# Chen-Suyi/PointRegGPT

Measured on AMD Instinct MI355X. Metric: generated point-cloud pairs/sec (node), 128x128 depth, 1000-step DDNM, higher is better.
Workload: dtype bf16; 1 GPU; configs[2]: full pipeline (SE(3) z-buffer reproject + MaskUnet + DDNM sampler + MaskUnet + f64 unproject); batch_per_gpu=64, image_size=128, transitions=1000, sampler=ancestral-ddnm, unet_dim=64, streams=2, parallelism=scene-sharded x1, no collectives, hipgraph=one captured transition (U-Net + update), replayed per step

## Files before the change

pointreggpt_amd/csrc/conv_c64.hip:

```cpp
#include <atomic>
#include <cstdlib>

#include "conv.h"

namespace prg {

typedef __attribute__((ext_vector_type(8))) __bf16 c64_bf16x8;
typedef __attribute__((ext_vector_type(16))) float c64_f32x16;
typedef __attribute__((ext_vector_type(4))) unsigned int c64_u32x4;
typedef __attribute__((ext_vector_type(8))) _Float16 c64_f16x8;

namespace {

constexpr int TH = 8, TW = 32, HP = TW + 2, HALO = (TH + 2) * HP;
constexpr int ROWB = 144;
constexpr int NPT = 256;
constexpr int RPP = NPT / 8;
constexpr int KU = (HALO + RPP - 1) / RPP;
constexpr size_t AH_BYTES = (size_t)KU * RPP * ROWB;
constexpr size_t C64_LDS = 2 * AH_BYTES + 64 * sizeof(float);

__device__ inline float c64_lo(uint32_t w) { return __uint_as_float(w << 16); }
__device__ inline float c64_hi(uint32_t w) { return __uint_as_float(w & 0xffff0000u); }
__device__ inline uint32_t c64_pack(float a, float b) {
// ... 110 lines not shown
      for (int c = 0; c < 4; ++c) {
        const bf16_t* const wsrc = PRO == 3 ? reinterpret_cast<const bf16_t*>(L.w_f16) : L.w;
        const bf16_t* p = wsrc + ((size_t)(tap * d.kchunks + (c >> 1)) * d.CoutPad + wn * 32 + l31) * 32 + (c & 1) * 16 + hi * 8;
        wf[tap][c] = *reinterpret_cast<const c64_bf16x8*>(p);
      }
    float* const bias_lds = reinterpret_cast<float*>(smem + 2 * AH_BYTES);
    if (tid < 64) bias_lds[tid] = L.bias[tid];
    const float* const biasp = bias_lds + wn * 32 + 4 * hi;
    const int gn_per = fuse_stats ? (64 / L.gn_groups) >> 3 : 1;
    const unsigned x0off = (unsigned)(((wm * 4) * HP + l31) * ROWB + hi * 16);
    auto mma = [](const c64_bf16x8& a, const c64_bf16x8& b, const c64_f32x16& c) -> c64_f32x16 {
      if constexpr (PRO == 3)
        return __builtin_amdgcn_mfma_f32_32x32x16_f16(__builtin_bit_cast(c64_f16x8, a), __builtin_bit_cast(c64_f16x8, b), c, 0, 0, 0);
      else
        return __builtin_amdgcn_mfma_f32_32x32x16_bf16(a, b, c, 0, 0, 0);
    };
    c64_barrier();
    for (int s = 0; s < nsteps; ++s) {
      const char* const xb = smem + (size_t)(s & 1) * AH_BYTES + x0off;
      c64_f32x16 acc[4];
#pragma unroll
      for (int q = 0; q < 4; ++q) {
        const float4 b4 = *reinterpret_cast<const float4*>(biasp + 8 * q);
#pragma unroll
        for (int pt = 0; pt < 4; ++pt) { acc[pt][4 * q] = b4.x; acc[pt][4 * q + 1] = b4.y; acc[pt][4 * q + 2] = b4.z; acc[pt][4 * q + 3] = b4.w; }
      }
      constexpr int FD = 3, FR = 4, NF = 72;
      c64_bf16x8 fr[FR];
      auto foff = [](int n) { return ((n / 12) * HP + (n / 4) % 3) * ROWB + (n & 3) * 32; };
#pragma unroll
      for (int j = 0; j < FD && j < NF; ++j) fr[j] = *reinterpret_cast<const c64_bf16x8*>(xb + foff(j));
#pragma unroll
      for (int n = 0; n < NF; ++n) {
        const int r = n / 12, dx = (n / 4) % 3, c = n & 3;
        if (n + FD < NF) fr[(n + FD) % FR] = *reinterpret_cast<const c64_bf16x8*>(xb + foff(n + FD));
#pragma unroll
        for (int dy = 0; dy < 3; ++dy) {
          const int pt = r - dy;
          if (pt >= 0 && pt < 4) acc[pt] = mma(wf[dy * 3 + dx][c], fr[n % FR], acc[pt]);
        }
        __builtin_amdgcn_sched_barrier(0);
      }
      int tb, ty0, tx0;
      c64_tile(first + s * stride, tiles_x, tiles_y, tb, ty0, tx0);
      if (fuse_stats && L.gn_tickets) asm volatile("s_waitcnt vmcnt(0)" ::: "memory");
      c64_barrier();
      float V[8];
#pragma unroll
      for (int q = 0; q < 4; ++q) {
        V[q] = 0.0f;
        V[4 + q] = 0.0f;
      }
      char* const obase = reinterpret_cast<char*>(L.out) +
                          ((((size_t)tb * d.Hout + ty0 + wm * 4) * d.Wout + tx0 + l31) * 64 + wn * 32 + 8 * hi) * 2;
      const size_t orow = (size_t)d.Wout * 128;
#pragma unroll
      for (int pt = 0; pt < 4; ++pt) {
        uint32_t pk[8];
#pragma unroll
        for (int q = 0; q < 4; ++q) {
          float v[4];
#pragma unroll
          for (int r = 0; r < 4; ++r) {
            v[r] = acc[pt][4 * q + r];
            V[q] += v[r];
            V[4 + q] = fmaf(v[r], v[r], V[4 + q]);
          }
          pk[2 * q] = O16 ? h16_pack(v[0], v[1]) : c64_pack(v[0], v[1]);
          pk[2 * q + 1] = O16 ? h16_pack(v[2], v[3]) : c64_pack(v[2], v[3]);
        }
#pragma unroll
        for (int m = 0; m < 2; ++m) {
          const auto s0 = __builtin_amdgcn_permlane32_swap(pk[4 * m], pk[4 * m + 2], false, false);
          const auto s1 = __builtin_amdgcn_permlane32_swap(pk[4 * m + 1], pk[4 * m + 3], false, false);
          const c64_u32x4 o = {(uint32_t)s0[0], (uint32_t)s1[0], (uint32_t)s0[1], (uint32_t)s1[1]};
          *reinterpret_cast<c64_u32x4*>(obase + pt * orow + m * 32) = o;
        }
      }
      if (fuse_stats) {
        const bool b0 = lane & 1, b1 = lane & 2, b2 = lane & 4;
        float A4[4], B2[2];
#pragma unroll
        for (int j = 0; j < 4; ++j) A4[j] = (b0 ? V[4 + j] : V[j]) + c64_dpp<0xB1>(b0 ? V[j] : V[4 + j]);
#pragma unroll
        for (int j = 0; j < 2; ++j) B2[j] = (b1 ? A4[2 + j] : A4[j]) + c64_dpp<0x4E>(b1 ? A4[j] : A4[2 + j]);
        float D = (b2 ? B2[1] : B2[0]) + c64_swz<4>(b2 ? B2[0] : B2[1]);
        D += c64_swz<8>(D);
        D += c64_swz<16>(D);
        D += __shfl_xor(D, 32, 64);
        const int per = gn_per > 4 ? 4 : gn_per;
        if (per >= 2) D += c64_swz<4>(D);
        if (per >= 4) D += c64_dpp<0x4E>(D);
        const int i = (lane & 1) * 4 + (lane & 2) + ((lane >> 2) & 1);
        const int q = i & 3;
        if (lane < 8 && (q & (per - 1)) == 0) {
          const int split_n = gn_per > 4 ? 2 : 1;
          const int nsplit = tiles_x * tiles_y * 2 * split_n;
          const int slab = (((ty0 / TH) * tiles_x + tx0 / TW) * 2 + wm) * split_n + (split_n == 2 ? wn : 0);
          const int grp = (wn * 4 + q) / gn_per;
          if (L.gn_acc) {
            int which = i >> 2;
            asm volatile("" : "+v"(which));
            gn_acc_add(L.gn_acc, L.gn_groups, tb, grp, which, D);
          } else {
            __hip_atomic_store(&L.gn_partials[(((size_t)tb * nsplit + slab) * L.gn_groups + grp) * 2 + (i >> 2)], D,
                               __ATOMIC_RELAXED, __HIP_MEMORY_SCOPE_AGENT);
          }
        }
      }
    }
    if (fuse_stats && L.gn_tickets) asm volatile("s_waitcnt vmcnt(0)" ::: "memory");
    if (nsteps & 1) c64_barrier();
    c64_barrier();
    return;
  }

  {
    const int ptid = tid - 256;
    const int slot = ptid & 7, row = ptid >> 3;
    char* const ah = smem + row * ROWB + slot * 16;
    const int Hl = d.Hout, Wl = d.Wout;
    int voffk[KU];
    unsigned m_valid = 0, m_top = 0, m_bot = 0, m_left = 0, m_right = 0;
#pragma unroll
    for (int k = 0; k < KU; ++k) {
      const int hp = k * RPP + row;
      const int hy = hp / HP, hx = hp - hy * HP;
      const bool valid = hp < HALO;
      const int dy = (hy - 1) >> d.ups, dx = (hx - 1) >> d.ups;
      voffk[k] = ((dy + 1) * d.Win + dx + 1) * 128 + slot * 16;
      m_valid |= (valid ? 1u : 0u) << k;
      m_top |= (valid && hy == 0 ? 1u : 0u) << k;
      m_bot |= (valid && hy == TH + 1 ? 1u : 0u) << k;
      m_left |= (valid && hx == 0 ? 1u : 0u) << k;
      m_right |= (valid && hx == HP - 1 ? 1u : 0u) << k;
    }
    const unsigned pad_bytes = (unsigned)(d.Win + 1) * 128u;
    const __amdgpu_buffer_rsrc_t rsrc = __builtin_amdgcn_make_buffer_rsrc(
        const_cast<char*>(reinterpret_cast<const char*>(L.src0)) - pad_bytes, 0,
        (int)((size_t)d.B * d.Hin * d.Win * 128 + pad_bytes), 0x00020000);
    c64_u32x4 hA[KU], hB[KU];
    const int tpi = tiles_x * tiles_y;
    int done_in_img = 0;
    unsigned okmask = 0, okmask_nxt = 0;
    float4 ca[2], cb[2], ca_n[2], cb_n[2];
    h16x2 ah2[4], bh2[4];
    longlong2 fs_n = make_longlong2(0, 0);
    auto issue = [&](int s, c64_u32x4(&h)[KU]) {
      int b, y0, x0;
      c64_tile(first + min(s, nsteps - 1) * stride, tiles_x, tiles_y, b, y0, x0);
      okmask_nxt = m_valid & ~((y0 == 0 ? m_top : 0u) | (y0 + TH == Hl ? m_bot : 0u) | (x0 == 0 ? m_left : 0u) |
                               (x0 + TW == Wl ? m_right : 0u));
      const int soff = __builtin_amdgcn_readfirstlane((((b * d.Hin + (y0 >> d.ups)) * d.Win) + (x0 >> d.ups)) * 128);
#pragma unroll
      for (int k = 0; k < KU; ++k)
        h[k] = __builtin_amdgcn_raw_buffer_load_b128(rsrc, ((okmask_nxt >> k) & 1u) ? voffk[k] : -1, soff, 0);
      if constexpr (PRO == 1) {
        const float* pa = L.pro_a + (size_t)b * 64 + slot * 8;
        const float* pb = L.pro_b + (size_t)b * 64 + slot * 8;
        ca_n[0] = *reinterpret_cast<const float4*>(pa);
        ca_n[1] = *reinterpret_cast<const float4*>(pa + 4);
        cb_n[0] = *reinterpret_cast<const float4*>(pb);
        cb_n[1] = *reinterpret_cast<const float4*>(pb + 4);
      }
      if constexpr (PRO >= 2) {
        const GnFold& f = L.pro_fold;
        fs_n = *reinterpret_cast<const longlong2*>(f.acc + ((size_t)b * f.G + (slot * 8) / f.cpg) * 2);
        const float* pp = f.P + (size_t)b * f.pq_stride + slot * 8;
        const float* pq = f.Q + (size_t)b * f.pq_stride + slot * 8;
        ca_n[0] = *reinterpret_cast<const float4*>(pp);
        ca_n[1] = *reinterpret_cast<const float4*>(pp + 4);
        cb_n[0] = *reinterpret_cast<const float4*>(pq);
        cb_n[1] = *reinterpret_cast<const float4*>(pq + 4);
      }
    };
    auto write = [&](int s, c64_u32x4(&h)[KU]) {
      char* dst = ah + (size_t)(s & 1) * AH_BYTES;
      const float a8[8] = {ca[0].x, ca[0].y, ca[0].z, ca[0].w, ca[1].x, ca[1].y, ca[1].z, ca[1].w};
      const float b8[8] = {cb[0].x, cb[0].y, cb[0].z, cb[0].w, cb[1].x, cb[1].y, cb[1].z, cb[1].w};
#pragma unroll
      for (int k = 0; k < KU; ++k) {
        c64_u32x4 v = h[k];
        if constexpr (PRO == 3) {
          v = h16_silu8(v, ah2, bh2);
        } else if constexpr (PRO) {
#pragma unroll
          for (int j = 0; j < 4; ++j) {
            const float lo = c64_silu(fmaf(c64_lo(v[j]), a8[2 * j], b8[2 * j]));
            const float hh = c64_silu(fmaf(c64_hi(v[j]), a8[2 * j + 1], b8[2 * j + 1]));
            v[j] = c64_pack(lo, hh);
          }
        }
        if constexpr (PRO != 0) {
          if (!((okmask >> k) & 1u)) v = c64_u32x4{0u, 0u, 0u, 0u};
        }
        *reinterpret_cast<c64_u32x4*>(dst + k * RPP * ROWB) = v;
      }
    };
    auto adopt = [&]() {
      okmask = okmask_nxt;
      if constexpr (PRO == 1) {
        ca[0] = ca_n[0]; ca[1] = ca_n[1]; cb[0] = cb_n[0]; cb[1] = cb_n[1];
      }
      if constexpr (PRO >= 2) {
        float mean, rstd;
        gn_fold_stats_raw(fs_n.x, fs_n.y, L.pro_fold.inv_n, mean, rstd);
#pragma unroll
        for (int h2 = 0; h2 < 2; ++h2) {
          ca[h2] = make_float4(rstd * ca_n[h2].x, rstd * ca_n[h2].y, rstd * ca_n[h2].z, rstd * ca_n[h2].w);
          cb[h2] = make_float4(fmaf(-mean, ca[h2].x, cb_n[h2].x), fmaf(-mean, ca[h2].y, cb_n[h2].y),
                               fmaf(-mean, ca[h2].z, cb_n[h2].z), fmaf(-mean, ca[h2].w, cb_n[h2].w));
        }
        if constexpr (PRO == 3) {
          typedef __attribute__((ext_vector_type(2))) float f32x2;
#pragma unroll
          for (int h2 = 0; h2 < 2; ++h2) {
            ah2[2 * h2] = __builtin_convertvector((f32x2){ca[h2].x, ca[h2].y}, h16x2);
            ah2[2 * h2 + 1] = __builtin_convertvector((f32x2){ca[h2].z, ca[h2].w}, h16x2);
            bh2[2 * h2] = __builtin_convertvector((f32x2){cb[h2].x, cb[h2].y}, h16x2);
            bh2[2 * h2 + 1] = __builtin_convertvector((f32x2){cb[h2].z, cb[h2].w}, h16x2);
          }
        }
      }
    };
    issue(0, hA);
    adopt();
    write(0, hA);
    issue(1, hB);
    c64_barrier();
    auto ticket = [&](int s) {
      if (fuse_stats && L.gn_tickets && ptid < 64) {
        const int t = first + s * stride;
        const int img = t / tpi;
        ++done_in_img;
        const bool leave = s + 1 == nsteps || (t + stride) / tpi != img;
        if (leave) {
          int old = 0;
          if (ptid == 0) old = __hip_atomic_fetch_add(L.gn_tickets + img, done_in_img, __ATOMIC_RELAXED, __HIP_MEMORY_SCOPE_AGENT);
          old = __builtin_amdgcn_readfirstlane(old);
          if (old + done_in_img == tpi) {
            if (ptid == 0) __hip_atomic_store(L.gn_tickets + img, 0, __ATOMIC_RELAXED, __HIP_MEMORY_SCOPE_AGENT);
            c64_fold_coefficients(L, img, tpi * 2 * (((64 / L.gn_groups) >> 3) > 4 ? 2 : 1), ptid);
          }
          done_in_img = 0;
        }
      }
    };
    const int n2 = (nsteps + 1) & ~1;
#pragma unroll 1
    for (int s = 0; s < n2; s += 2) {
      adopt();
      issue(s + 2, hA);
      write(s + 1, hB);
      c64_barrier();
      if (s > 0) ticket(s - 1);
      adopt();
      issue(s + 3, hB);
      write(s + 2, hA);
      c64_barrier();
      if (s < nsteps) ticket(s);
    }
    c64_barrier();
    if (n2 == nsteps) ticket(nsteps - 1);
  }
}

}

int try_launch_conv3x3_c64(const ConvLaunch<bf16_t>& L, hipStream_t s, int* gn_nsplit_out, int* acc_done) {
  static const int enabled = env_int("PRG_CONV_C64", 1);
  if (!enabled) return 0;
  const ConvDesc& d = L.d;
  if (!(d.KH == 3 && d.KW == 3 && d.stride == 1 && d.pad == 1)) return 0;
  if (d.C0 != 64 || d.C1 != 0 || d.Cout != 64 || d.CoutPad != 64 || d.kchunks != 2) return 0;
  if (L.residual || !L.bias) return 0;
  if (d.ups) return 0;
  if (d.Wout % TW || d.Hout % TH) return 0;
  if ((size_t)d.B * d.Hin * d.Win * 128 + 4096 >= ((size_t)1 << 31)) return 0;
  const int tiles_x = d.Wout / TW, tiles_y = d.Hout / TH;
  const int total = tiles_x * tiles_y * d.B;
  const int num_cus = device_cu_count();
  if (num_cus <= 0) return 0;
  int grid = (total < num_cus ? total : num_cus) & ~7;
  if (grid < 8) return 0;
  const int cpg = L.gn_groups > 0 ? 64 / L.gn_groups : 0;
  const int split_n = cpg > 32 ? 2 : 1;
  int fuse = L.gn_partials != nullptr && cpg % 8 == 0 && cpg <= 64 && (cpg & (cpg - 1)) == 0 &&
             tiles_x * tiles_y * 2 * split_n <= kGnMaxSplit;
  if (L.gn_partials && !fuse) return 0;
  static DeviceOnce attr_done[5];
  const GnFold& pf = L.pro_fold;
  const bool fold_ok = pf.acc && pf.P && pf.Q && pf.G * pf.cpg == 64 && pf.cpg % 8 == 0;
  if (pf.acc && !fold_ok) return 0;
  if (L.in_f16 && !(fold_ok && L.w_f16)) return 0;
  const int pro = L.in_f16 ? 3 : fold_ok ? 2 : (L.pro_a ? 1 : 0);
  if (L.out_f16 && pro != 0) return 0;
  const int variant = L.out_f16 ? 4 : pro;
  const void* const fns[5] = {reinterpret_cast<const void*>(&conv3x3_c64_kernel<0, false>), reinterpret_cast<const void*>(&conv3x3_c64_kernel<1, false>),
                              reinterpret_cast<const void*>(&conv3x3_c64_kernel<2, false>), reinterpret_cast<const void*>(&conv3x3_c64_kernel<3, false>),
                              reinterpret_cast<const void*>(&conv3x3_c64_kernel<0, true>)};
  if (!attr_done[variant].done()) {
    hipError_t e = hipFuncSetAttribute(fns[variant], hipFuncAttributeMaxDynamicSharedMemorySize, (int)C64_LDS);
    if (e != hipSuccess) return fail(PRG_E_HIP, std::string("hipFuncSetAttribute(c64 conv): ") + hipGetErrorString(e));
    attr_done[variant].mark();
  }
  if (gn_nsplit_out) *gn_nsplit_out = fuse ? tiles_x * tiles_y * 2 * split_n : 0;
  const bool use_acc = fuse && L.gn_acc != nullptr;
  ConvLaunch<bf16_t> Lk = L;
  Lk.gn_tickets = nullptr;
  if (!use_acc) Lk.gn_acc = nullptr;
  if (acc_done) *acc_done = use_acc ? 1 : 0;
  const int flags = (fuse ? 1 : 0) | 2;
  if (L.probe) return 1;
  if (variant == 4) conv3x3_c64_kernel<0, true><<<dim3(grid), 512, C64_LDS, s>>>(Lk, tiles_x, tiles_y, flags);
  else if (pro == 3) conv3x3_c64_kernel<3, false><<<dim3(grid), 512, C64_LDS, s>>>(Lk, tiles_x, tiles_y, flags);
  else if (pro == 2) conv3x3_c64_kernel<2, false><<<dim3(grid), 512, C64_LDS, s>>>(Lk, tiles_x, tiles_y, flags);
  else if (pro == 1) conv3x3_c64_kernel<1, false><<<dim3(grid), 512, C64_LDS, s>>>(Lk, tiles_x, tiles_y, flags);
  else conv3x3_c64_kernel<0, false><<<dim3(grid), 512, C64_LDS, s>>>(Lk, tiles_x, tiles_y, flags);
  PRG_LAUNCH_CHECK();
  return 1;
}

}
```

pointreggpt_amd/csrc/conv_ws.hip:

```cpp
#include <atomic>

#include "conv.h"

namespace prg {

typedef __attribute__((ext_vector_type(8))) __bf16 bf16x8;
typedef __attribute__((ext_vector_type(16))) float f32x16;
typedef __attribute__((ext_vector_type(4))) unsigned int u32x4;

namespace {

constexpr int kCH = 64;

__device__ inline float bf_lo(uint32_t w) { return __uint_as_float(w << 16); }
__device__ inline float bf_hi(uint32_t w) { return __uint_as_float(w & 0xffff0000u); }
__device__ inline uint32_t pack_bf16(float a, float b) {
  typedef __attribute__((ext_vector_type(2))) __bf16 bf16x2;
  bf16x2 v = {(__bf16)a, (__bf16)b};
  return __builtin_bit_cast(uint32_t, v);
}
template <int CTRL>
__device__ inline float dpp_f32(float v) {
  return __builtin_bit_cast(float, __builtin_amdgcn_update_dpp(0, __builtin_bit_cast(int, v), CTRL, 0xF, 0xF, false));
}
template <int XOR>
__device__ inline float swz_xor(float v) {
  return __builtin_bit_cast(float, __builtin_amdgcn_ds_swizzle(__builtin_bit_cast(int, v), (XOR << 10) | 0x1F));
}
__device__ inline float fast_silu(float x) {
  return x * __builtin_amdgcn_rcpf(1.0f + __builtin_amdgcn_exp2f(x * -1.4426950408889634f));
}

template <bool LDS_DONE = true>
__device__ __forceinline__ void phase_barrier() {
  if constexpr (LDS_DONE) asm volatile("s_waitcnt lgkmcnt(0)" ::: "memory");
  __builtin_amdgcn_s_barrier();
  asm volatile("" ::: "memory");
}

template <int TH, int TW, int BN>
struct WsGeom {
  static constexpr int BM = TH * TW;
  static constexpr int HP = TW + 2;
  static constexpr int HALO = (TH + 2) * HP;
  static constexpr int WAVES_N = BN / 64, WAVES_M = 4 / WAVES_N;
  static constexpr int ROWB = 144;
  static constexpr size_t AH_BYTES = (size_t)HALO * ROWB;
  static constexpr size_t BW_BYTES = (size_t)BN * ROWB;
  static constexpr size_t RED_BYTES = 0;
  static constexpr size_t STG_BYTES = 4 * 64 * 128;
  static constexpr size_t BIAS_BYTES = BN * sizeof(float);
  static constexpr size_t LDS = 2 * AH_BYTES + 3 * BW_BYTES + RED_BYTES + STG_BYTES + BIAS_BYTES;
  static_assert(LDS <= 160 * 1024, "LDS budget");
  static_assert(BM / WAVES_M == 64, "consumer wave tile is 64 pixels x 64 channels");
};

struct TileCur { int n, x, y, b; };

struct TileMap {
  int tiles_x, tiles_y, tiles_n, TH, TW;
  int pinned, tn_fixed;
  int first, stride, count;
  TileCur c0, dc;

  __device__ __forceinline__ void digits(int t, TileCur& c) const {
    if (pinned) {
      c.n = 0;
    } else {
      c.n = t % tiles_n;
      t /= tiles_n;
    }
    c.x = t % tiles_x; t /= tiles_x;
    c.y = t % tiles_y;
    c.b = t / tiles_y;
  }
  __device__ __forceinline__ void next(TileCur& c) const {
    int carry = 0;
    if (!pinned) {
      c.n += dc.n;
      if (c.n >= tiles_n) { c.n -= tiles_n; carry = 1; }
    }
    c.x += dc.x + carry; carry = 0;
    if (c.x >= tiles_x) { c.x -= tiles_x; carry = 1; }
    c.y += dc.y + carry; carry = 0;
    if (c.y >= tiles_y) { c.y -= tiles_y; carry = 1; }
    c.b += dc.b + carry;
  }
  __device__ __forceinline__ void fill(const TileCur& c, int& b, int& y0, int& x0, int& tn) const {
    b = c.b; y0 = c.y * TH; x0 = c.x * TW;
    tn = pinned ? tn_fixed : c.n;
  }

  __device__ __forceinline__ void init(int bid, int GR, int tx, int ty, int tn, int nb, int th, int tw) {
    tiles_x = tx; tiles_y = ty; tiles_n = tn; TH = th; TW = tw;
    const int npix = tx * ty * nb;
    const bool xcd_ok = (GR & 7) == 0;
    const int per_xcd = GR >> 3;
    const int xcd = bid & 7, idx = bid >> 3;
    if (xcd_ok && tn > 1 && (8 % tn) == 0) {
      pinned = 1;
      tn_fixed = xcd % tn;
      const int gx = 8 / tn, member = xcd / tn;
      first = member * per_xcd + idx;
      stride = gx * per_xcd;
      count = first < npix ? (npix - first + stride - 1) / stride : 0;
    } else {
      pinned = 0;
      tn_fixed = 0;
      first = xcd_ok ? xcd * per_xcd + idx : bid;
      stride = GR;
      const int total = npix * tn;
      count = first < total ? (total - first + stride - 1) / stride : 0;
    }
    digits(first, c0);
    digits(stride, dc);
  }
  __device__ __forceinline__ void decode(int it, int& b, int& y0, int& x0, int& tn) const {
    int t = first + it * stride;
    if (pinned) {
      tn = tn_fixed;
    } else {
      tn = t % tiles_n;
      t /= tiles_n;
    }
    const int tx = t % tiles_x; t /= tiles_x;
    const int ty = t % tiles_y;
    b = t / tiles_y;
    y0 = ty * TH; x0 = tx * TW;
  }
};

template <int TH, int TW, int BN, bool PRO>
struct Producer {
  using G = WsGeom<TH, TW, BN>;
  static constexpr int HP = G::HP, HALO = G::HALO;
  static constexpr int NPT = 512;
  static constexpr int NWL = BN * 8 / NPT;
  static constexpr int RPP = NPT / 8;
  static constexpr int DRAIN_PHASES = 2048 / NPT;
  static constexpr int KU = (HALO + RPP - 1) / RPP;
  static constexpr int UPH = (KU + 7) / 8 > 2 ? (KU + 7) / 8 : 2;
  static constexpr int NCO = PRO ? 4 : 0;
  static constexpr int PER_STEP = 9 * NWL + KU + NCO;
  static constexpr int U_YOUNGER = PER_STEP - 1;
  static_assert(U_YOUNGER <= 63, "vmcnt range");
  static constexpr int n_units(int p) {
    p = ((p % 9) + 9) % 9;
    if (p == 8) return 0;
    const int lo = p * UPH, hi = (p + 1) * UPH < KU ? (p + 1) * UPH : KU;
    return hi > lo ? hi - lo : 0;
  }
  static constexpr int n_coef(int p) { return ((p % 9) + 9) % 9 == 0 ? NCO : 0; }
  static constexpr int WD = 6;
  static constexpr int w_younger(int ph) {
    int n = n_units(ph - WD) + n_coef(ph);
    for (int j = 1; j < WD; ++j) n += n_coef(ph - j) + NWL + n_units(ph - j);
    return n;
  }
  static_assert(9 % 3 == 0 && 18 % WD == 0, "set index must be a compile-time function of (g & 1, phase)");

  const ConvLaunch<bf16_t>& L;
  const ConvDesc& d;
  const TileMap& tm;
  char* Ah0;
  char* Bw0;
  u32x4 wset[WD][NWL];
  u32x4 hreg[KU];
  u32x4 cf[2][4];
  unsigned hpix[KU];
  unsigned w_voff;
  unsigned cf_voff;
  unsigned dr_voff;
  unsigned hedge[KU];
  unsigned hvalid, hvalid_nxt;
  const char* ld_base;
  unsigned ld_cs2;
  unsigned ld_dummy;
  const char* ld_ca;
  const char* ld_cb;
  unsigned ld_tedge;
  int slot, row, nsteps, nchunks, Hl, Wl;
  struct StepInfo { int chunk, b, y0, x0, tn; TileCur cur; };
  StepInfo sA, sB, sC, dr;
  int gC;
  bool drain_on;
  const char* wptr;
  size_t w_tapb;
  char* dr_base;
  size_t dr_rowb;
  char* stage_rd;
  int dr_r0;

  __device__ __forceinline__ Producer(const ConvLaunch<bf16_t>& L_, char* smem, int ptid, const TileMap& tm_, int nsteps_,
                                      int nchunks_)
      : L(L_), d(L_.d), tm(tm_), nsteps(nsteps_), nchunks(nchunks_) {
    Ah0 = smem + (ptid >> 3) * G::ROWB + (ptid & 7) * 16;
    Bw0 = smem + 2 * G::AH_BYTES + (ptid >> 3) * G::ROWB + (ptid & 7) * 16;
    slot = ptid & 7;
    row = ptid >> 3;
    Hl = d.Hout;
    Wl = d.Wout;
    hvalid = hvalid_nxt = 0;
    ld_ca = ld_cb = nullptr;
    drain_on = false;
    w_tapb = (size_t)d.kchunks * d.CoutPad * 64;
    dr_rowb = (size_t)d.Wout * d.Cout * 2;
    dr_base = nullptr;
    wptr = nullptr;
    dr_r0 = ptid >> 3;
    stage_rd = smem + 2 * G::AH_BYTES + 3 * G::BW_BYTES + G::RED_BYTES + dr_r0 * 128 + (((ptid & 7) ^ ((dr_r0 >> 1) & 7)) << 4);
    sA.chunk = 0;
    sA.cur = tm.c0;
    tm.fill(sA.cur, sA.b, sA.y0, sA.x0, sA.tn);
    sB = sA; gC = 0;
    advance(sB);
    sC = sB;
    advance(sC);
    dr = sA;
    w_voff = (unsigned)((((slot >> 2) * d.CoutPad + row) * 32 + (slot & 3) * 8) * 2);
    cf_voff = (unsigned)(slot * 8 * 4);
    dr_voff = (unsigned)((((dr_r0 / TW) * d.Wout + dr_r0 % TW) * d.Cout + slot * 8) * 2);
    ld_dummy = (unsigned)((d.Win + 1));
#pragma unroll
    for (int k = 0; k < KU; ++k) {
      const int hp = k * RPP + row;
      const int hy = hp / HP, hx = hp - hy * HP;
      int ry = hy - 1, rx = hx - 1;
      if (d.ups) { ry >>= 1; rx >>= 1; }
      hpix[k] = (unsigned)((ry + 1) * d.Win + (rx + 1));
      hedge[k] = (hy == 0 ? 1u : 0u) | (hy == TH + 1 ? 2u : 0u) | (hx == 0 ? 4u : 0u) | (hx == TW + 1 ? 8u : 0u) |
                 (hp >= HALO ? 16u : 0u);
    }
  }

  __device__ __forceinline__ void advance(StepInfo& si) {
    if (gC + 1 < nsteps) {
      ++gC;
      if (++si.chunk == nchunks) {
        si.chunk = 0;
        tm.next(si.cur);
        tm.fill(si.cur, si.b, si.y0, si.x0, si.tn);
      }
    }
  }
  __device__ __forceinline__ const char* w_tile(int tap, int chunk, int tn) const {
    return reinterpret_cast<const char*>(L.w) + ((size_t)(tap * d.kchunks + 2 * chunk) * d.CoutPad + tn * BN) * 64;
  }
  template <int SET>
  __device__ __forceinline__ void w_issue(const char* base) {
    asm volatile("global_load_dwordx4 %0, %1, %2" : "=v"(wset[SET][0]) : "v"(w_voff), "s"(base) : "memory");
    if constexpr (NWL == 2) {
      const char* base2 = base + 4096;
      asm volatile("global_load_dwordx4 %0, %1, %2" : "=v"(wset[SET][NWL - 1]) : "v"(w_voff), "s"(base2) : "memory");
    }
  }
  template <int SET, int N>
  __device__ __forceinline__ void w_wait() {
    if constexpr (NWL == 2)
      asm volatile("s_waitcnt vmcnt(%[n])" : "+v"(wset[SET][0]), "+v"(wset[SET][1]) : [n] "i"(N) : "memory");
    else
      asm volatile("s_waitcnt vmcnt(%[n])" : "+v"(wset[SET][0]) : [n] "i"(N) : "memory");
    static_assert(NWL == 2 || NWL == 1, "weight units per thread");
  }
  template <int SET>
  __device__ __forceinline__ void w_write(int ring) {
#pragma unroll
    for (int j = 0; j < NWL; ++j)
      *reinterpret_cast<u32x4*>(Bw0 + ring * G::BW_BYTES + j * 64 * G::ROWB) = wset[SET][j];
  }

  __device__ __forceinline__ void issue_setup(const StepInfo& si) {
    const int b = si.b, y0 = si.y0, x0 = si.x0, chunk = si.chunk;
    const int c = chunk * kCH;
    const bool first = c < d.C0;
    const bf16_t* src = first ? L.src0 : L.src1;
    const int cs = first ? d.C0 : d.C1;
    const int cc = first ? c : c - d.C0;
    ld_cs2 = (unsigned)(cs * 2);
    ld_tedge = (y0 == 0 ? 1u : 0u) | (y0 + TH == Hl ? 2u : 0u) | (x0 == 0 ? 4u : 0u) | (x0 + TW == Wl ? 8u : 0u) | 16u;
    const int64_t horg = ((int64_t)b * d.Hin + (y0 >> d.ups)) * d.Win + (x0 >> d.ups) - (d.Win + 1);
    ld_base = reinterpret_cast<const char*>(src) + (horg * cs + cc) * 2;
    if constexpr (PRO) {
      const size_t o = ((size_t)b * d.C0 + chunk * kCH) * 4;
      ld_ca = reinterpret_cast<const char*>(L.pro_a) + o;
      ld_cb = reinterpret_cast<const char*>(L.pro_b) + o;
    }
    hvalid_nxt = 0;
  }
  template <int CS>
  __device__ __forceinline__ void issue_coeffs() {
    if constexpr (PRO) {
      asm volatile("global_load_dwordx4 %0, %1, %2" : "=v"(cf[CS][0]) : "v"(cf_voff), "s"(ld_ca) : "memory");
      asm volatile("global_load_dwordx4 %0, %1, %2 offset:16" : "=v"(cf[CS][1]) : "v"(cf_voff), "s"(ld_ca) : "memory");
      asm volatile("global_load_dwordx4 %0, %1, %2" : "=v"(cf[CS][2]) : "v"(cf_voff), "s"(ld_cb) : "memory");
      asm volatile("global_load_dwordx4 %0, %1, %2 offset:16" : "=v"(cf[CS][3]) : "v"(cf_voff), "s"(ld_cb) : "memory");
    }
  }
  template <int K>
  __device__ __forceinline__ void issue_unit() {
    const bool ok = (hedge[K] & ld_tedge) == 0;
    const unsigned pix = ok ? hpix[K] : ld_dummy;
    const unsigned voff = __umul24(pix, ld_cs2) + (unsigned)(slot * 16);
    asm volatile("global_load_dwordx4 %0, %1, %2" : "=v"(hreg[K]) : "v"(voff), "s"(ld_base) : "memory");
    hvalid_nxt |= (ok ? 1u : 0u) << K;
  }
  template <int K, int CS, int N>
  __device__ __forceinline__ void wait_unit() {
    if constexpr (PRO) {
      asm volatile("s_waitcnt vmcnt(%[n])"
                   : "+v"(hreg[K]), "+v"(cf[CS][0]), "+v"(cf[CS][1]), "+v"(cf[CS][2]), "+v"(cf[CS][3])
                   : [n] "i"(N)
                   : "memory");
    } else {
      asm volatile("s_waitcnt vmcnt(%[n])" : "+v"(hreg[K]) : [n] "i"(N) : "memory");
    }
  }
  template <int K, int CS>
  __device__ __forceinline__ void write_unit(int g_tgt, bool wr) {
    const int hp = K * RPP + row;
    if (hp < HALO && wr) {
      u32x4 v = hreg[K];
      if constexpr (PRO) {
#pragma unroll
        for (int j = 0; j < 4; ++j) {
          const float a_lo = __uint_as_float(cf[CS][j >> 1][(2 * j) & 3]);
          const float a_hi = __uint_as_float(cf[CS][j >> 1][((2 * j) & 3) + 1]);
          const float b_lo = __uint_as_float(cf[CS][2 + (j >> 1)][(2 * j) & 3]);
          const float b_hi = __uint_as_float(cf[CS][2 + (j >> 1)][((2 * j) & 3) + 1]);
          const float lo = fast_silu(fmaf(bf_lo(v[j]), a_lo, b_lo));
          const float hi2 = fast_silu(fmaf(bf_hi(v[j]), a_hi, b_hi));
          v[j] = pack_bf16(lo, hi2);
        }
      }
      if (!((hvalid >> K) & 1u)) v = u32x4{0u, 0u, 0u, 0u};
      *reinterpret_cast<u32x4*>(Ah0 + (g_tgt & 1) * G::AH_BYTES + K * RPP * G::ROWB) = v;
    }
  }
  template <int PH>
  __device__ __forceinline__ u32x4 drain_read() {
    return *reinterpret_cast<const u32x4*>(stage_rd + PH * 8192);
  }
  template <int PH>
  __device__ __forceinline__ void drain_store(const u32x4& v) {
    constexpr int wm = PH / G::WAVES_N, wn = PH % G::WAVES_N;
    constexpr int prow = (wm * 64) / TW;
    char* base = dr_base + prow * dr_rowb + wn * 128;
    asm volatile("global_store_dwordx4 %0, %1, %2" ::"v"(dr_voff), "v"(v), "s"(base) : "memory");
  }
  template <int PH>
  __device__ __forceinline__ void drain_unit() {
    drain_store<PH>(drain_read<PH>());
  }
  template <int PH, int J, int CSW>
  __device__ __forceinline__ void units_wait() {
    if constexpr (J < UPH && PH * UPH + J < KU) {
      wait_unit<PH * UPH + J, CSW, U_YOUNGER - NWL - J>();
      units_wait<PH, J + 1, CSW>();
    }
  }
  template <int PH, int J, int CSW>
  __device__ __forceinline__ void units_write(int g, bool wr) {
    if constexpr (J < UPH && PH * UPH + J < KU) {
      write_unit<PH * UPH + J, CSW>(g + 1, wr);
      units_write<PH, J + 1, CSW>(g, wr);
    }
  }
  template <int PH, int J>
  __device__ __forceinline__ void units_issue() {
    if constexpr (J < UPH && PH * UPH + J < KU) {
      issue_unit<PH * UPH + J>();
      units_issue<PH, J + 1>();
    }
  }
  template <int GP, int PH, bool LIVE>
  __device__ __forceinline__ void phase(int g, bool wr, int chunk0, int tn0, int chunk1, int tn1) {
    constexpr int SET = (3 * GP + PH + 2) % WD;
    constexpr int RING = (PH + 2) % 3;
    u32x4 dv;
    bool draining = false;
    if constexpr (LIVE && PH < DRAIN_PHASES) {
      draining = drain_on;
      if (draining) dv = drain_read<PH>();
    }
    if constexpr (LIVE || PH >= WD) {
      w_wait<SET, w_younger(PH)>();
      w_write<SET>(RING);
    }
    if constexpr (LIVE && PH < 8) {
      units_wait<PH, 0, (GP + 1) & 1>();
      units_write<PH, 0, (GP + 1) & 1>(g, wr);
    }
    constexpr int TAPN = PH + 2 + WD;
    static_assert(TAPN < 18, "weight prefetch reaches at most into the next step");
    if constexpr (!LIVE) wptr = TAPN < 9 ? w_tile(TAPN, chunk0, tn0) : w_tile(TAPN - 9, chunk1, tn1);
    else if constexpr (TAPN == 9) wptr = w_tile(0, chunk1, tn1);
    else wptr += w_tapb;
    w_issue<SET>(wptr);
    if constexpr (PH < 8) units_issue<PH, 0>();
    if constexpr (LIVE && PH < DRAIN_PHASES) {
      if (draining) drain_store<PH>(dv);
    }
    if constexpr (LIVE) phase_barrier();
  }
  template <int GP, bool LIVE>
  __device__ __forceinline__ void step(int g) {
    const bool wr = g + 1 < nsteps;
    if constexpr (LIVE) {
      const int c0 = sA.chunk, t0 = sA.tn, c1 = sB.chunk, t1 = sB.tn;
      drain_on = g > 0 && sA.chunk == 0;
      issue_coeffs<GP>();
      phase<GP, 0, LIVE>(g, wr, c0, t0, c1, t1); phase<GP, 1, LIVE>(g, wr, c0, t0, c1, t1);
      phase<GP, 2, LIVE>(g, wr, c0, t0, c1, t1); phase<GP, 3, LIVE>(g, wr, c0, t0, c1, t1);
      phase<GP, 4, LIVE>(g, wr, c0, t0, c1, t1); phase<GP, 5, LIVE>(g, wr, c0, t0, c1, t1);
      phase<GP, 6, LIVE>(g, wr, c0, t0, c1, t1); phase<GP, 7, LIVE>(g, wr, c0, t0, c1, t1);
      hvalid = hvalid_nxt;
      dr = sA;
      dr_base = reinterpret_cast<char*>(L.out) +
                ((((int64_t)dr.b * Hl + dr.y0) * Wl + dr.x0) * d.Cout + dr.tn * BN) * 2;
      sA = sB;
      sB = sC;
      advance(sC);
      issue_setup(sC);
      phase<GP, 8, LIVE>(g, wr, c0, t0, c1, t1);
    } else {
      const int c0 = sA.chunk, t0 = sA.tn;
      issue_setup(sB);
      issue_coeffs<GP>();
      phase<GP, 0, LIVE>(g, wr, c0, t0, c0, t0); phase<GP, 1, LIVE>(g, wr, c0, t0, c0, t0);
      phase<GP, 2, LIVE>(g, wr, c0, t0, c0, t0); phase<GP, 3, LIVE>(g, wr, c0, t0, c0, t0);
      phase<GP, 4, LIVE>(g, wr, c0, t0, c0, t0); phase<GP, 5, LIVE>(g, wr, c0, t0, c0, t0);
      phase<GP, 6, LIVE>(g, wr, c0, t0, c0, t0); phase<GP, 7, LIVE>(g, wr, c0, t0, c0, t0);
      phase<GP, 8, LIVE>(g, wr, c0, t0, c0, t0);
      hvalid = hvalid_nxt;
      issue_setup(sC);
    }
  }
  template <int K>
  __device__ __forceinline__ void prologue_issue() {
    if constexpr (K < KU) {
      issue_unit<K>();
      prologue_issue<K + 1>();
    }
  }
  template <int K>
  __device__ __forceinline__ void prologue_write() {
    if constexpr (K < KU) {
      wait_unit<K, 0, 0>();
      write_unit<K, 0>(0, true);
      prologue_write<K + 1>();
    }
  }
  __device__ __forceinline__ void prologue() {
    issue_setup(sA);
    issue_coeffs<0>();
    prologue_issue<0>();
    hvalid = hvalid_nxt;
    prologue_write<0>();
    step<1, false>(-1);
  }
  template <int K>
  __device__ __forceinline__ void keep_units() {
    if constexpr (K < KU) {
      asm volatile("" : "+v"(hreg[K])::"memory");
      keep_units<K + 1>();
    }
  }
  __device__ __forceinline__ void finish() {
    drain_unit<0>(); drain_unit<1>(); drain_unit<2>(); drain_unit<3>();
    static_assert(DRAIN_PHASES == 4, "one consumer wave's stage per drain phase");
    asm volatile("s_waitcnt vmcnt(0)" ::: "memory");
#pragma unroll
    for (int sidx = 0; sidx < WD; ++sidx)
#pragma unroll
      for (int j = 0; j < NWL; ++j) asm volatile("" : "+v"(wset[sidx][j])::"memory");
    keep_units<0>();
    if constexpr (PRO) {
#pragma unroll
      for (int c = 0; c < 2; ++c)
#pragma unroll
        for (int j = 0; j < 4; ++j) asm volatile("" : "+v"(cf[c][j])::"memory");
    }
    phase_barrier();
  }
};

template <int TH, int TW, int BN, bool PRO>
__global__ __launch_bounds__(768) void conv3x3_ws_kernel(const ConvLaunch<bf16_t> L, const int tiles_x,
                                                            const int tiles_y, const int tiles_n, const int fuse_stats) {
  using G = WsGeom<TH, TW, BN>;
  constexpr int HP = G::HP;
  extern __shared__ __attribute__((aligned(16))) char smem[];
  constexpr int ROWB = G::ROWB;
  char* const stage = smem + 2 * G::AH_BYTES + 3 * G::BW_BYTES + G::RED_BYTES;
  float* const bias_lds = reinterpret_cast<float*>(stage + G::STG_BYTES);

  const ConvDesc& d = L.d;
  const int tid = threadIdx.x, wave = tid >> 6, lane = tid & 63;
  const int nchunks = (d.C0 + d.C1) / kCH;
  TileMap tmap;
  tmap.init((int)blockIdx.x, (int)gridDim.x, tiles_x, tiles_y, tiles_n, d.B, TH, TW);
  const int my_tiles = tmap.count;
  const int nsteps = my_tiles * nchunks;
  if (nsteps == 0) return;

  if (wave < 4) {
    __builtin_amdgcn_s_setprio(3);
    const int gn_per = fuse_stats ? (d.Cout / L.gn_groups) >> 3 : 1;
    const int gn_per_sh = 31 - __builtin_clz(gn_per);
    const int wm = wave / G::WAVES_N, wn = wave % G::WAVES_N;
    const int l31 = lane & 31, hi = lane >> 5;
    const int lpx = (TW == 16 && l31 >= 16) ? 16 + ((l31 - 2) & 15) : l31;
    const char* xrow[2];
    const char* wrowp[2];
#pragma unroll
    for (int pt = 0; pt < 2; ++pt) {
      const int p = wm * 64 + pt * 32 + lpx;
      xrow[pt] = smem + ((p / TW) * HP + (p % TW)) * ROWB + hi * 16;
    }
#pragma unroll
    for (int ct = 0; ct < 2; ++ct) wrowp[ct] = smem + 2 * G::AH_BYTES + (wn * 64 + ct * 32 + l31) * ROWB + hi * 16;
    f32x16 acc[2][2];
#pragma unroll
    for (int ct = 0; ct < 2; ++ct)
#pragma unroll
      for (int pt = 0; pt < 2; ++pt)
#pragma unroll
        for (int e = 0; e < 16; ++e) acc[ct][pt][e] = 0.0f;

    if (tid < BN) bias_lds[tid] = L.bias[(tmap.pinned ? tmap.tn_fixed : 0) * BN + tid];
    phase_barrier<true>();
    bf16x8 fw[3][2], fx[3][2];
    const char* xa[2] = {xrow[0], xrow[1]};
    const char* xn[2] = {xrow[0] + G::AH_BYTES, xrow[1] + G::AH_BYTES};
#define PRG_LW(SET, CT, RING, CALL) fw[SET][CT] = *reinterpret_cast<const bf16x8*>(wrowp[CT] + (RING) * (int)G::BW_BYTES + (CALL) * 32)
#define PRG_LX(SET, PT, BASE, TOFF, CALL) fx[SET][PT] = *reinterpret_cast<const bf16x8*>(BASE[PT] + (TOFF) * ROWB + (CALL) * 32)
#define PRG_MM(SET, CT, PT) acc[CT][PT] = __builtin_amdgcn_mfma_f32_32x32x16_bf16(fw[SET][CT], fx[SET][PT], acc[CT][PT], 0, 0, 0)
#define PRG_SB() __builtin_amdgcn_sched_barrier(0)
    PRG_LW(0, 0, 0, 0); PRG_LX(0, 0, xa, 0, 0); PRG_LX(0, 1, xa, 0, 0); PRG_LW(0, 1, 0, 0);
    PRG_LW(1, 0, 0, 1); PRG_LX(1, 0, xa, 0, 1); PRG_LX(1, 1, xa, 0, 1); PRG_LW(1, 1, 0, 1);
    int chunk = 0, it = 0;
    int tb = 0, ty0 = 0, tx0 = 0, ttn = 0;
    TileCur tcur = tmap.c0;
    tmap.fill(tcur, tb, ty0, tx0, ttn);
    for (int g = 0; g < nsteps; ++g) {
      const bool tile_end = chunk == nchunks - 1;
#pragma unroll
      for (int p = 0; p < 9; ++p) {
        const int toff = (p / 3) * HP + (p % 3);
        const int pn = p == 8 ? 0 : p + 1;
        const int toffN = (pn / 3) * HP + (pn % 3);
#pragma unroll
        for (int call = 0; call < 4; ++call) {
          const int sl = (4 * p + call + 2) % 3, sm = (4 * p + call) % 3;
          if (call < 2) {
            PRG_LW(sl, 0, p % 3, call + 2); PRG_MM(sm, 0, 0); PRG_SB();
            PRG_LX(sl, 0, xa, toff, call + 2); PRG_MM(sm, 0, 1); PRG_SB();
            PRG_LX(sl, 1, xa, toff, call + 2); PRG_MM(sm, 1, 0); PRG_SB();
            PRG_LW(sl, 1, p % 3, call + 2); PRG_MM(sm, 1, 1); PRG_SB();
          } else if (p == 8) {
            PRG_LW(sl, 0, (p + 1) % 3, call - 2); PRG_MM(sm, 0, 0); PRG_SB();
            PRG_LX(sl, 0, xn, toffN, call - 2); PRG_MM(sm, 0, 1); PRG_SB();
            PRG_LX(sl, 1, xn, toffN, call - 2); PRG_MM(sm, 1, 0); PRG_SB();
            PRG_LW(sl, 1, (p + 1) % 3, call - 2); PRG_MM(sm, 1, 1); PRG_SB();
          } else {
            PRG_LW(sl, 0, (p + 1) % 3, call - 2); PRG_MM(sm, 0, 0); PRG_SB();
            PRG_LX(sl, 0, xa, toffN, call - 2); PRG_MM(sm, 0, 1); PRG_SB();
            PRG_LX(sl, 1, xa, toffN, call - 2); PRG_MM(sm, 1, 0); PRG_SB();
            PRG_LW(sl, 1, (p + 1) % 3, call - 2); PRG_MM(sm, 1, 1); PRG_SB();
          }
        }
        if (p == 8 && tile_end) {
          char* const stg = stage + wave * (64 * 128);
          float V[16];
          const bool o16 = L.out_f16 != 0;
#pragma unroll
          for (int ct = 0; ct < 2; ++ct)
#pragma unroll
            for (int q = 0; q < 4; ++q) {
              const float4 b4 = *reinterpret_cast<const float4*>(bias_lds + wn * 64 + ct * 32 + 8 * q + 4 * hi);
              const float bv[4] = {b4.x, b4.y, b4.z, b4.w};
              float s = 0.0f, sq = 0.0f;
#pragma unroll
              for (int pt = 0; pt < 2; ++pt) {
                float v[4];
#pragma unroll
                for (int r = 0; r < 4; ++r) {
                  v[r] = acc[ct][pt][4 * q + r] + bv[r];
                  s += v[r];
                  sq = fmaf(v[r], v[r], sq);
                }
                uint2 w;
                w.x = o16 ? h16_pack(v[0], v[1]) : pack_bf16(v[0], v[1]);
                w.y = o16 ? h16_pack(v[2], v[3]) : pack_bf16(v[2], v[3]);
                const int px = pt * 32 + lpx;
                *reinterpret_cast<uint2*>(stg + px * 128 + (((ct * 4 + q) ^ ((px >> 1) & 7)) << 4) + hi * 8) = w;
              }
              V[ct * 4 + q] = s;
              V[8 + ct * 4 + q] = sq;
            }
          if (fuse_stats) {
            const bool b0 = lane & 1, b1 = lane & 2, b2 = lane & 4, b3 = lane & 8;
            float A8[8], B4[4], C2[2];
#pragma unroll
            for (int j = 0; j < 8; ++j) A8[j] = (b0 ? V[8 + j] : V[j]) + dpp_f32<0xB1>(b0 ? V[j] : V[8 + j]);
#pragma unroll
            for (int j = 0; j < 4; ++j) B4[j] = (b1 ? A8[4 + j] : A8[j]) + dpp_f32<0x4E>(b1 ? A8[j] : A8[4 + j]);
#pragma unroll
            for (int j = 0; j < 2; ++j) C2[j] = (b2 ? B4[2 + j] : B4[j]) + swz_xor<4>(b2 ? B4[j] : B4[2 + j]);
            float D = (b3 ? C2[1] : C2[0]) + swz_xor<8>(b3 ? C2[0] : C2[1]);
            D += swz_xor<16>(D);
            D += __shfl_xor(D, 32, 64);
            const int per = gn_per;
            if (per >= 2) D += swz_xor<8>(D);
            if (per >= 4) D += swz_xor<4>(D);
            if (per >= 8) D += dpp_f32<0x4E>(D);
            const int i = (lane & 1) * 8 + (lane & 2) * 2 + ((lane >> 2) & 1) * 2 + ((lane >> 3) & 1);
            const int cc = i & 7;
            if (lane < 16 && (cc & (per - 1)) == 0) {
              const int nsplit = tiles_x * tiles_y * G::WAVES_M;
              const int slab = ((ty0 / TH) * tiles_x + tx0 / TW) * G::WAVES_M + wm;
              const int grp = (((ttn * BN + wn * 64) >> 3) + cc) >> gn_per_sh;
              if (L.gn_acc) gn_acc_add(L.gn_acc, L.gn_groups, tb, grp, i >> 3, D);
              else L.gn_partials[(((size_t)tb * nsplit + slab) * L.gn_groups + grp) * 2 + (i >> 3)] = D;
            }
          }
#pragma unroll
          for (int ct = 0; ct < 2; ++ct)
#pragma unroll
            for (int pt = 0; pt < 2; ++pt)
#pragma unroll
              for (int e = 0; e < 16; ++e) acc[ct][pt][e] = 0.0f;
        }
        if (p == 8 && tile_end) phase_barrier<true>();
        else phase_barrier<false>();
      }
      { const char* t0 = xa[0]; xa[0] = xn[0]; xn[0] = t0; const char* t1 = xa[1]; xa[1] = xn[1]; xn[1] = t1; }
      if (++chunk == nchunks) {
        chunk = 0;
        if (++it < my_tiles) {
          tmap.next(tcur);
          tmap.fill(tcur, tb, ty0, tx0, ttn);
        }
      }
    }
#undef PRG_LW
#undef PRG_LX
#undef PRG_MM
#undef PRG_SB
    phase_barrier<false>();
    return;
  }

  {
    Producer<TH, TW, BN, PRO> Pv(L, smem, tid - 256, tmap, nsteps, nchunks);
    Pv.prologue();
    phase_barrier();
#pragma unroll 1
    for (int g = 0; g < nsteps; g += 2) {
      Pv.template step<0, true>(g);
      if (g + 1 < nsteps) Pv.template step<1, true>(g + 1);
    }
    Pv.finish();
  }
}

constexpr int kWsUnsupported = 100;

template <int TH, int TW, int BN, bool PRO>
int launch_ws_cfg2(const ConvLaunch<bf16_t>& L, hipStream_t s, int fuse_stats, int* nsplit, int num_cus) {
  using G = WsGeom<TH, TW, BN>;
  const ConvDesc& d = L.d;
  const int tiles_x = d.Wout / TW, tiles_y = d.Hout / TH, tiles_n = d.Cout / BN;
  const int total = tiles_x * tiles_y * tiles_n * d.B;
  int grid = num_cus;
  if (grid > total) grid = total;
  if (grid >= 8) grid &= ~7;
  if (tiles_n > 1 && (grid & 7) != 0) return kWsUnsupported;
  static DeviceOnce attr_done;
  if (!attr_done.done()) {
    hipError_t e = hipFuncSetAttribute(reinterpret_cast<const void*>(&conv3x3_ws_kernel<TH, TW, BN, PRO>),
                                       hipFuncAttributeMaxDynamicSharedMemorySize, (int)G::LDS);
    if (e != hipSuccess) return fail(PRG_E_HIP, std::string("hipFuncSetAttribute(ws conv): ") + hipGetErrorString(e));
    attr_done.mark();
  }
  if (nsplit) *nsplit = fuse_stats ? tiles_x * tiles_y * G::WAVES_M : 0;
  if (L.probe) return PRG_OK;
  conv3x3_ws_kernel<TH, TW, BN, PRO><<<dim3(grid), 768, G::LDS, s>>>(L, tiles_x, tiles_y, tiles_n, fuse_stats);
  PRG_LAUNCH_CHECK();
  return PRG_OK;
}

template <int TH, int TW, int BN>
int launch_ws_cfg(const ConvLaunch<bf16_t>& L, hipStream_t s, int fuse_stats, int* nsplit, int num_cus) {
  return L.pro_a ? launch_ws_cfg2<TH, TW, BN, true>(L, s, fuse_stats, nsplit, num_cus)
                 : launch_ws_cfg2<TH, TW, BN, false>(L, s, fuse_stats, nsplit, num_cus);
}

}

int try_launch_conv3x3_ws(const ConvLaunch<bf16_t>& L, hipStream_t s, int* gn_nsplit_out, int* acc_done) {
  static const int enabled = env_int("PRG_CONV_WS", 1);
  if (!enabled) return 0;
  const ConvDesc& d = L.d;
  if (!(d.KH == 3 && d.KW == 3 && d.stride == 1 && d.pad == 1)) return 0;
  if (d.C0 % kCH || d.C1 % kCH || d.Cout % 64) return 0;
  if (L.residual || !L.bias) return 0;
  if (L.in_f16 || (L.out_f16 && L.pro_a)) return 0;
  {
    const int tn128 = d.Cout % 128 == 0 ? d.Cout / 128 : d.Cout / 64;
    if (tn128 != 1 && tn128 != 2 && tn128 != 4 && tn128 != 8) return 0;
  }
  const int num_cus = device_cu_count();
  if (num_cus <= 0) return 0;
  const int H = d.Hout, W = d.Wout;
  const int cpg = L.gn_groups > 0 ? d.Cout / L.gn_groups : 0;
  const bool want = L.gn_partials != nullptr;
  auto fuse_for = [&](int TH, int TW, int BN) {
    return want && cpg % 8 == 0 && cpg <= 64 && (cpg & (cpg - 1)) == 0 && (W / TW) * (H / TH) * (4 / (BN / 64)) <= kGnMaxSplit ? 1 : 0;
  };
  int rc = 0;
  if (d.Cout % 128 == 0) {
    if (W % 32 == 0 && H % 4 == 0) rc = launch_ws_cfg<4, 32, 128>(L, s, fuse_for(4, 32, 128), gn_nsplit_out, num_cus);
    else if (W % 16 == 0 && H % 8 == 0) rc = launch_ws_cfg<8, 16, 128>(L, s, fuse_for(8, 16, 128), gn_nsplit_out, num_cus);
    else return 0;
  } else {
    if (W % 32 == 0 && H % 8 == 0) rc = launch_ws_cfg<8, 32, 64>(L, s, fuse_for(8, 32, 64), gn_nsplit_out, num_cus);
    else return 0;
  }
  if (rc == kWsUnsupported) return 0;
  if (rc == PRG_OK && acc_done) *acc_done = (L.gn_acc && gn_nsplit_out && *gn_nsplit_out > 0) ? 1 : 0;
  return rc == PRG_OK ? 1 : rc;
}

}
```

Measured before the change: 14.55 pairs/s.

## Store conv epilogue directly from consumer waves via permlane32 swap, drop producer LDS drain

The warp-specialized conv epilogue used to stage bf16 outputs in an LDS buffer, which producer threads then drained to global memory over later phases. Consumer waves now pack their outputs, exchange halves across the wave with permlane32_swap, and write 16-byte chunks straight to global memory. This frees the staging LDS and removes the drain logic and the extra LDS wait at tile end. The trade is that consumers now spend time on global stores. Separately, the c64 kernel issues its halo buffer loads after the coefficient loads instead of before.

```diff
diff --git a/pointreggpt_amd/csrc/conv_c64.hip b/pointreggpt_amd/csrc/conv_c64.hip
--- a/pointreggpt_amd/csrc/conv_c64.hip
+++ b/pointreggpt_amd/csrc/conv_c64.hip
@@ -286,9 +286,6 @@
       okmask_nxt = m_valid & ~((y0 == 0 ? m_top : 0u) | (y0 + TH == Hl ? m_bot : 0u) | (x0 == 0 ? m_left : 0u) |
                                (x0 + TW == Wl ? m_right : 0u));
       const int soff = __builtin_amdgcn_readfirstlane((((b * d.Hin + (y0 >> d.ups)) * d.Win) + (x0 >> d.ups)) * 128);
-#pragma unroll
-      for (int k = 0; k < KU; ++k)
-        h[k] = __builtin_amdgcn_raw_buffer_load_b128(rsrc, ((okmask_nxt >> k) & 1u) ? voffk[k] : -1, soff, 0);
       if constexpr (PRO == 1) {
         const float* pa = L.pro_a + (size_t)b * 64 + slot * 8;
         const float* pb = L.pro_b + (size_t)b * 64 + slot * 8;
@@ -307,6 +304,9 @@
         cb_n[0] = *reinterpret_cast<const float4*>(pq);
         cb_n[1] = *reinterpret_cast<const float4*>(pq + 4);
       }
+#pragma unroll
+      for (int k = 0; k < KU; ++k)
+        h[k] = __builtin_amdgcn_raw_buffer_load_b128(rsrc, ((okmask_nxt >> k) & 1u) ? voffk[k] : -1, soff, 0);
     };
     auto write = [&](int s, c64_u32x4(&h)[KU]) {
       char* dst = ah + (size_t)(s & 1) * AH_BYTES;
diff --git a/pointreggpt_amd/csrc/conv_ws.hip b/pointreggpt_amd/csrc/conv_ws.hip
--- a/pointreggpt_amd/csrc/conv_ws.hip
+++ b/pointreggpt_amd/csrc/conv_ws.hip
@@ -47,10 +47,8 @@
   static constexpr int ROWB = 144;
   static constexpr size_t AH_BYTES = (size_t)HALO * ROWB;
   static constexpr size_t BW_BYTES = (size_t)BN * ROWB;
-  static constexpr size_t RED_BYTES = 0;
-  static constexpr size_t STG_BYTES = 4 * 64 * 128;
   static constexpr size_t BIAS_BYTES = BN * sizeof(float);
-  static constexpr size_t LDS = 2 * AH_BYTES + 3 * BW_BYTES + RED_BYTES + STG_BYTES + BIAS_BYTES;
+  static constexpr size_t LDS = 2 * AH_BYTES + 3 * BW_BYTES + BIAS_BYTES;
   static_assert(LDS <= 160 * 1024, "LDS budget");
   static_assert(BM / WAVES_M == 64, "consumer wave tile is 64 pixels x 64 channels");
 };
@@ -137,7 +135,6 @@
   static constexpr int NPT = 512;
   static constexpr int NWL = BN * 8 / NPT;
   static constexpr int RPP = NPT / 8;
-  static constexpr int DRAIN_PHASES = 2048 / NPT;
   static constexpr int KU = (HALO + RPP - 1) / RPP;
   static constexpr int UPH = (KU + 7) / 8 > 2 ? (KU + 7) / 8 : 2;
   static constexpr int NCO = PRO ? 4 : 0;
@@ -170,7 +167,6 @@
   unsigned hpix[KU];
   unsigned w_voff;
   unsigned cf_voff;
-  unsigned dr_voff;
   unsigned hedge[KU];
   unsigned hvalid, hvalid_nxt;
   const char* ld_base;
@@ -181,15 +177,10 @@
   unsigned ld_tedge;
   int slot, row, nsteps, nchunks, Hl, Wl;
   struct StepInfo { int chunk, b, y0, x0, tn; TileCur cur; };
-  StepInfo sA, sB, sC, dr;
+  StepInfo sA, sB, sC;
   int gC;
-  bool drain_on;
   const char* wptr;
   size_t w_tapb;
-  char* dr_base;
-  size_t dr_rowb;
-  char* stage_rd;
-  int dr_r0;
 
   __device__ __forceinline__ Producer(const ConvLaunch<bf16_t>& L_, char* smem, int ptid, const TileMap& tm_, int nsteps_,
                                       int nchunks_)
@@ -202,13 +193,8 @@
     Wl = d.Wout;
     hvalid = hvalid_nxt = 0;
     ld_ca = ld_cb = nullptr;
-    drain_on = false;
     w_tapb = (size_t)d.kchunks * d.CoutPad * 64;
-    dr_rowb = (size_t)d.Wout * d.Cout * 2;
-    dr_base = nullptr;
     wptr = nullptr;
-    dr_r0 = ptid >> 3;
-    stage_rd = smem + 2 * G::AH_BYTES + 3 * G::BW_BYTES + G::RED_BYTES + dr_r0 * 128 + (((ptid & 7) ^ ((dr_r0 >> 1) & 7)) << 4);
     sA.chunk = 0;
     sA.cur = tm.c0;
     tm.fill(sA.cur, sA.b, sA.y0, sA.x0, sA.tn);
@@ -216,10 +202,8 @@
     advance(sB);
     sC = sB;
     advance(sC);
-    dr = sA;
     w_voff = (unsigned)((((slot >> 2) * d.CoutPad + row) * 32 + (slot & 3) * 8) * 2);
     cf_voff = (unsigned)(slot * 8 * 4);
-    dr_voff = (unsigned)((((dr_r0 / TW) * d.Wout + dr_r0 % TW) * d.Cout + slot * 8) * 2);
     ld_dummy = (unsigned)((d.Win + 1));
 #pragma unroll
     for (int k = 0; k < KU; ++k) {
@@ -336,21 +320,6 @@
       *reinterpret_cast<u32x4*>(Ah0 + (g_tgt & 1) * G::AH_BYTES + K * RPP * G::ROWB) = v;
     }
   }
-  template <int PH>
-  __device__ __forceinline__ u32x4 drain_read() {
-    return *reinterpret_cast<const u32x4*>(stage_rd + PH * 8192);
-  }
-  template <int PH>
-  __device__ __forceinline__ void drain_store(const u32x4& v) {
-    constexpr int wm = PH / G::WAVES_N, wn = PH % G::WAVES_N;
-    constexpr int prow = (wm * 64) / TW;
-    char* base = dr_base + prow * dr_rowb + wn * 128;
-    asm volatile("global_store_dwordx4 %0, %1, %2" ::"v"(dr_voff), "v"(v), "s"(base) : "memory");
-  }
-  template <int PH>
-  __device__ __forceinline__ void drain_unit() {
-    drain_store<PH>(drain_read<PH>());
-  }
   template <int PH, int J, int CSW>
   __device__ __forceinline__ void units_wait() {
     if constexpr (J < UPH && PH * UPH + J < KU) {
@@ -376,12 +345,6 @@
   __device__ __forceinline__ void phase(int g, bool wr, int chunk0, int tn0, int chunk1, int tn1) {
     constexpr int SET = (3 * GP + PH + 2) % WD;
     constexpr int RING = (PH + 2) % 3;
-    u32x4 dv;
-    bool draining = false;
-    if constexpr (LIVE && PH < DRAIN_PHASES) {
-      draining = drain_on;
-      if (draining) dv = drain_read<PH>();
-    }
     if constexpr (LIVE || PH >= WD) {
       w_wait<SET, w_younger(PH)>();
       w_write<SET>(RING);
@@ -397,9 +360,6 @@
     else wptr += w_tapb;
     w_issue<SET>(wptr);
     if constexpr (PH < 8) units_issue<PH, 0>();
-    if constexpr (LIVE && PH < DRAIN_PHASES) {
-      if (draining) drain_store<PH>(dv);
-    }
     if constexpr (LIVE) phase_barrier();
   }
   template <int GP, bool LIVE>
@@ -407,16 +367,12 @@
     const bool wr = g + 1 < nsteps;
     if constexpr (LIVE) {
       const int c0 = sA.chunk, t0 = sA.tn, c1 = sB.chunk, t1 = sB.tn;
-      drain_on = g > 0 && sA.chunk == 0;
       issue_coeffs<GP>();
       phase<GP, 0, LIVE>(g, wr, c0, t0, c1, t1); phase<GP, 1, LIVE>(g, wr, c0, t0, c1, t1);
       phase<GP, 2, LIVE>(g, wr, c0, t0, c1, t1); phase<GP, 3, LIVE>(g, wr, c0, t0, c1, t1);
       phase<GP, 4, LIVE>(g, wr, c0, t0, c1, t1); phase<GP, 5, LIVE>(g, wr, c0, t0, c1, t1);
       phase<GP, 6, LIVE>(g, wr, c0, t0, c1, t1); phase<GP, 7, LIVE>(g, wr, c0, t0, c1, t1);
       hvalid = hvalid_nxt;
-      dr = sA;
-      dr_base = reinterpret_cast<char*>(L.out) +
-                ((((int64_t)dr.b * Hl + dr.y0) * Wl + dr.x0) * d.Cout + dr.tn * BN) * 2;
       sA = sB;
       sB = sC;
       advance(sC);
@@ -466,8 +422,6 @@
     }
   }
   __device__ __forceinline__ void finish() {
-    drain_unit<0>(); drain_unit<1>(); drain_unit<2>(); drain_unit<3>();
-    static_assert(DRAIN_PHASES == 4, "one consumer wave's stage per drain phase");
     asm volatile("s_waitcnt vmcnt(0)" ::: "memory");
 #pragma unroll
     for (int sidx = 0; sidx < WD; ++sidx)
@@ -491,8 +445,7 @@
   constexpr int HP = G::HP;
   extern __shared__ __attribute__((aligned(16))) char smem[];
   constexpr int ROWB = G::ROWB;
-  char* const stage = smem + 2 * G::AH_BYTES + 3 * G::BW_BYTES + G::RED_BYTES;
-  float* const bias_lds = reinterpret_cast<float*>(stage + G::STG_BYTES);
+  float* const bias_lds = reinterpret_cast<float*>(smem + 2 * G::AH_BYTES + 3 * G::BW_BYTES);
 
   const ConvDesc& d = L.d;
   const int tid = threadIdx.x, wave = tid >> 6, lane = tid & 63;
@@ -512,10 +465,12 @@
     const int lpx = (TW == 16 && l31 >= 16) ? 16 + ((l31 - 2) & 15) : l31;
     const char* xrow[2];
     const char* wrowp[2];
+    unsigned opix[2];
 #pragma unroll
     for (int pt = 0; pt < 2; ++pt) {
       const int p = wm * 64 + pt * 32 + lpx;
       xrow[pt] = smem + ((p / TW) * HP + (p % TW)) * ROWB + hi * 16;
+      opix[pt] = (unsigned)(((p / TW) * d.Wout + (p % TW)) * d.Cout * 2 + hi * 16);
     }
 #pragma unroll
     for (int ct = 0; ct < 2; ++ct) wrowp[ct] = smem + 2 * G::AH_BYTES + (wn * 64 + ct * 32 + l31) * ROWB + hi * 16;
@@ -570,33 +525,38 @@
           }
         }
         if (p == 8 && tile_end) {
-          char* const stg = stage + wave * (64 * 128);
           float V[16];
+#pragma unroll
+          for (int i = 0; i < 16; ++i) V[i] = 0.0f;
           const bool o16 = L.out_f16 != 0;
+          char* const obase = reinterpret_cast<char*>(L.out) +
+                              ((((size_t)tb * d.Hout + ty0) * d.Wout + tx0) * d.Cout + ttn * BN + wn * 64) * 2;
 #pragma unroll
           for (int ct = 0; ct < 2; ++ct)
 #pragma unroll
-            for (int q = 0; q < 4; ++q) {
-              const float4 b4 = *reinterpret_cast<const float4*>(bias_lds + wn * 64 + ct * 32 + 8 * q + 4 * hi);
-              const float bv[4] = {b4.x, b4.y, b4.z, b4.w};
-              float s = 0.0f, sq = 0.0f;
-#pragma unroll
-              for (int pt = 0; pt < 2; ++pt) {
+            for (int pt = 0; pt < 2; ++pt) {
+              uint32_t pk[8];
+#pragma unroll
+              for (int q = 0; q < 4; ++q) {
+                const float4 b4 = *reinterpret_cast<const float4*>(bias_lds + wn * 64 + ct * 32 + 8 * q + 4 * hi);
+                const float bv[4] = {b4.x, b4.y, b4.z, b4.w};
                 float v[4];
 #pragma unroll
                 for (int r = 0; r < 4; ++r) {
                   v[r] = acc[ct][pt][4 * q + r] + bv[r];
-                  s += v[r];
-                  sq = fmaf(v[r], v[r], sq);
+                  V[ct * 4 + q] += v[r];
+                  V[8 + ct * 4 + q] = fmaf(v[r], v[r], V[8 + ct * 4 + q]);
                 }
-                uint2 w;
-                w.x = o16 ? h16_pack(v[0], v[1]) : pack_bf16(v[0], v[1]);
-                w.y = o16 ? h16_pack(v[2], v[3]) : pack_bf16(v[2], v[3]);
-                const int px = pt * 32 + lpx;
-                *reinterpret_cast<uint2*>(stg + px * 128 + (((ct * 4 + q) ^ ((px >> 1) & 7)) << 4) + hi * 8) = w;
+                pk[2 * q] = o16 ? h16_pack(v[0], v[1]) : pack_bf16(v[0], v[1]);
+                pk[2 * q + 1] = o16 ? h16_pack(v[2], v[3]) : pack_bf16(v[2], v[3]);
               }
-              V[ct * 4 + q] = s;
-              V[8 + ct * 4 + q] = sq;
+#pragma unroll
+              for (int m = 0; m < 2; ++m) {
+                const auto s0 = __builtin_amdgcn_permlane32_swap(pk[4 * m], pk[4 * m + 2], false, false);
+                const auto s1 = __builtin_amdgcn_permlane32_swap(pk[4 * m + 1], pk[4 * m + 3], false, false);
+                const u32x4 o = {(uint32_t)s0[0], (uint32_t)s1[0], (uint32_t)s0[1], (uint32_t)s1[1]};
+                *reinterpret_cast<u32x4*>(obase + opix[pt] + ct * 64 + m * 32) = o;
+              }
             }
           if (fuse_stats) {
             const bool b0 = lane & 1, b1 = lane & 2, b2 = lane & 4, b3 = lane & 8;
@@ -631,8 +591,7 @@
 #pragma unroll
               for (int e = 0; e < 16; ++e) acc[ct][pt][e] = 0.0f;
         }
-        if (p == 8 && tile_end) phase_barrier<true>();
-        else phase_barrier<false>();
+        phase_barrier<false>();
       }
       { const char* t0 = xa[0]; xa[0] = xn[0]; xn[0] = t0; const char* t1 = xa[1]; xa[1] = xn[1]; xn[1] = t1; }
       if (++chunk == nchunks) {
```

Result: no change. 14.65 pairs/s (median of 6 runs) (+0.7%).
